# reinforcement-learning-kr/alpha_omok

Measured on AMD Instinct MI355X. Metric: self-play move-decisions/sec (9x9, 400 sims/move), higher is better.
Workload: dtype f32 (fp16x2-split MFMA operands, 3 products per multiply-add, f32 accumulate; inter-layer activations stored as two fp16 halves: ~22 significand bits)

## Files before the change

### alpha_omok_amd/csrc/net.hip

```cpp
#include <hip/hip_runtime.h>

#include <cmath>
#include <cstdio>
#include <cstdlib>
#include <cstring>
#include <map>
#include <type_traits>
#include <string>
#include <thread>
#include <vector>

#include "../../include/omok_hip.h"
#include "engine_types.hpp"
#include "host_handle.hpp"
#include "launchers.hpp"
#include "net_device.hpp"
#include "net_common.hpp"
#include "net_trunk_f32.hpp"
#include "net_trunk_h16.hpp"
#include "net_layer_ksplit.hpp"
#include "net_board_h16.hpp"
#include "net_small.hpp"
#include "net_w16.hpp"
#include "net_f16.hpp"
// ... 7 lines not shown
    int mode = 0;
    int requested_mode = 0;
    int fp16_fallbacks = 0;
    bool forced_fp32 = false;
    int num_cu = 256;
    bool finalized = false;
    std::map<std::string, std::vector<float>> params;
    ao::DevPool pool;
    std::vector<std::pair<void*, size_t>> pallocs;
    size_t pcursor = 0;
    std::vector<float*> conv_w, conv_sc, conv_sh;
    std::vector<uint4*> convh_wh, convh_wl;
    uint4 *step_w1h = nullptr, *step_w1l = nullptr;
    std::vector<float*> convh_sc;
    float* conv0_w16 = nullptr;
    float* conv0_w1 = nullptr;
    int nchq1 = 0;
    float *head_w3 = nullptr, *head_sc3 = nullptr, *head_sh3 = nullptr;
    float *wp_t = nullptr, *bp = nullptr, *w1_t = nullptr, *b1 = nullptr, *w2 = nullptr, *b2 = nullptr;
    int ws_boards = 0;
    float *act_x = nullptr, *act_t = nullptr, *hbuf = nullptr, *il_in = nullptr;
    float *tmp_p = nullptr, *tmp_v = nullptr;
    int* d_status = nullptr;
    bool attr_l[16][2] = {}, attr_done[16] = {}, lds_attr_done[16] = {}, attr_k[16] = {};
    int ksplit_min = 48, ksplit_max = 64, ksplit_max2 = 0;
    int rowk_min = 1, rowk_max = 47;
    bool attr_r[16] = {};
    int boardk_min = 64;
    bool attr_b[16] = {};
    long perboard_cells = 2592;
    int force_xt = 0, force_nch = 0;
    bool force_resident = false;
    ao::EventTimer timer{512};
    bool timing = false;
    int last_in_kind = 1;
    bool w16 = false;
    int products_req = 0;
    int precision_req = AO_NET_PRECISION_FP32;
    int trunk_fmt = -1;
};

template <typename T>
static int param_alloc(ao_net* n, T** out, size_t count) {
    const size_t bytes = std::max<size_t>(count * sizeof(T), 16);
    if (n->pcursor < n->pallocs.size() && n->pallocs[n->pcursor].second == bytes) {
        *out = static_cast<T*>(n->pallocs[n->pcursor++].first);
        return 0;
    }
    void* p = nullptr;
    hipError_t st = hipMalloc(&p, bytes);
    if (st != hipSuccess) return n->fail(std::string("hipMalloc(") + std::to_string(bytes) + " B): " + hipGetErrorString(st));
    n->pool.adopt(p);
    if (n->pcursor < n->pallocs.size()) {
        n->pool.release(n->pallocs[n->pcursor].first);
        n->pallocs[n->pcursor] = {p, bytes};
    } else {
        n->pallocs.push_back({p, bytes});
    }
    ++n->pcursor;
    *out = static_cast<T*>(p);
    return 0;
// ... 459 lines not shown
            hipLaunchKernelGGL(k_head_fc, dim3(boards), dim3(256), lds1, s, n->hbuf, n->wp_t, n->bp, n->w1_t, n->b1, n->w2, n->b2, policy, value,
                               n->A, n->planes);
            AO_HIP(n, hipGetLastError());
            return 0;
        } else {
            for (int l = 0; l <= 2 * n->nb; ++l)
                if (layer(l)) return 1;
        }
        AO_HIP(n, hipGetLastError());
        heads_h16 = f16l ? 2 : 1;
    } else if (group == 16 && mode == 5) {
        TrunkHArgs a;
        a.in0 = reinterpret_cast<const float4*>(in_il);
        a.bufA = reinterpret_cast<uint4*>(n->act_x);
        a.bufB = reinterpret_cast<uint4*>(n->act_t);
        a.nlayers = 1 + 2 * n->nb;
        a.CQ = n->CQ;
        a.COUT = n->planes;
        a.w3 = n->head_w3; a.sc3 = n->head_sc3; a.sh3 = n->head_sh3;
        a.wp_t = n->wp_t; a.bp = n->bp; a.w1_t = n->w1_t; a.b1 = n->b1; a.w2 = n->w2; a.b2 = n->b2;
        a.policy = policy;
        a.value = value;
        a.live = live; a.row_cap = row_cap;
        for (int l = 0; l < a.nlayers; ++l) {
            a.layers[l].wh = n->convh_wh[l];
            a.layers[l].wl = n->convh_wl[l];
            a.layers[l].sc = reinterpret_cast<const float4*>(n->convh_sc[l]);
            a.layers[l].sh = reinterpret_cast<const float4*>(n->conv_sh[l]);
            a.layers[l].ovf = n->d_status;
        }
        if (n->timing) n->timer.begin(s);
        if (fp16_forward(n)) {
            if (n->B > 9) return n->fail("split-fp16 trunk: board larger than 9x9");
            AO_HIP(n, ao::launch_trunk16h_f16(n->device, n->B, in_kind, groups, s, a));
        } else if (two_products(n) && n->trunk_fmt != 1) {
            if (n->B > 9) return n->fail("split-fp16 trunk: board larger than 9x9");
            AO_HIP(n, ao::launch_trunk16h_w16(n->device, n->B, in_kind, groups, s, a));
        } else
        switch (n->B) {
#define AO_BW_CASE(W)                                                                                        \
    case W: {                                                                                                \
        constexpr size_t heads_ = (static_cast<size_t>(3) * 128 + 16 * 3 * W * W + 8 * 16 * W * W + 8 * 16 * 128) * 4;  \
        constexpr size_t rows_ = static_cast<size_t>(2) * W * 4 * 2 * 1024 + 64;    \
        constexpr size_t lds_ = (rows_ > heads_) ? rows_ : heads_;                                            \
        if (!n->attr_done[W]) {                                                                                 \
            AO_HIP(n, hipFuncSetAttribute(reinterpret_cast<const void*>(&k_trunk16h<W, 4, 0>),              \
                                           hipFuncAttributeMaxDynamicSharedMemorySize, static_cast<int>(lds_))); \
            AO_HIP(n, hipFuncSetAttribute(reinterpret_cast<const void*>(&k_trunk16hb<W, 4, 0>),              \
                                           hipFuncAttributeMaxDynamicSharedMemorySize, static_cast<int>(lds_))); \
            AO_HIP(n, hipFuncSetAttribute(reinterpret_cast<const void*>(&k_trunk16h<W, 4, 1>),              \
                                           hipFuncAttributeMaxDynamicSharedMemorySize, static_cast<int>(lds_))); \
            AO_HIP(n, hipFuncSetAttribute(reinterpret_cast<const void*>(&k_trunk16hb<W, 4, 1>),              \
                                           hipFuncAttributeMaxDynamicSharedMemorySize, static_cast<int>(lds_))); \
            n->attr_done[W] = true;                                                                           \
        }                                                                                                    \
        if (n->trunk_fmt == 1) {                                                                             \
            if (in_kind == 2) hipLaunchKernelGGL((k_trunk16hb<W, 4, 1>), dim3(groups), dim3(512), lds_, s, a);    \
            else hipLaunchKernelGGL((k_trunk16h<W, 4, 1>), dim3(groups), dim3(512), lds_, s, a);                 \
        } else {                                                                                             \
            if (in_kind == 2) hipLaunchKernelGGL((k_trunk16hb<W, 4, 0>), dim3(groups), dim3(512), lds_, s, a);    \
            else hipLaunchKernelGGL((k_trunk16h<W, 4, 0>), dim3(groups), dim3(512), lds_, s, a);                 \
        }                                                                                                    \
    } break;
            AO_BW_CASE(3) AO_BW_CASE(4) AO_BW_CASE(5) AO_BW_CASE(6) AO_BW_CASE(7) AO_BW_CASE(8) AO_BW_CASE(9)
#undef AO_BW_CASE
            default: return n->fail("split-fp16 trunk: board larger than 9x9");
        }
        if (n->timing) n->timer.end(s);
        AO_HIP(n, hipGetLastError());
#ifdef AO_PROF
        if (getenv("AO_PROF_PRINT")) {
            unsigned long long h[96];
            hipStreamSynchronize(s);
            hipMemcpyFromSymbol(h, HIP_SYMBOL(ao_prof), sizeof(h));
            static const char* nm[12] = {"stage0", "slabs", "epilogue", "barrier", "last_epi+boundary", "heads", "conv1", "total",
                                         "s0:sync1", "s0:stage-issue", "s0:loads-land", "s0:sync2"};
            for (int k = 0; k < 12; ++k) {
                fprintf(stderr, "AO_PROF %-18s", nm[k]);
                for (int t = 0; t < 8; ++t) fprintf(stderr, " %9llu", h[t * 12 + k]);
// ... 118 lines not shown
    n->nchq16 = (((inplanes + 3) / 4) + 7) & ~7;
    n->nchq1 = (((inplanes + 3) / 4) + 3) & ~3;
    n->CQ = planes / 4;
    {
        hipDeviceProp_t prop;
        if (hipGetDeviceProperties(&prop, device) == hipSuccess && prop.multiProcessorCount > 0)
            n->num_cu = prop.multiProcessorCount;
    }
    if (const char* v = getenv("AO_KSPLIT")) {
        int lo = 0, hi = 0, hi2 = 0;
        if (sscanf(v, "%d,%d,%d", &lo, &hi, &hi2) == 3) { n->ksplit_min = lo > 0 ? lo : 1 << 30; n->ksplit_max = hi; n->ksplit_max2 = hi2; }
    }
    if (const char* v = getenv("AO_PERBOARD_CELLS")) n->perboard_cells = atol(v);
    if (const char* v = getenv("AO_BOARDK")) n->boardk_min = atoi(v);
    if (const char* v = getenv("AO_ROWK")) {
        int lo = 0, hi = -1;
        if (sscanf(v, "%d,%d", &lo, &hi) == 2) { n->rowk_min = lo; n->rowk_max = hi; }
    }
    if (const char* v = getenv("AO_TRUNK_FMT")) n->trunk_fmt = atoi(v) == 1 ? 1 : 0;
    if (n->trunk_fmt < 0) n->trunk_fmt = 0;
    if (const char* v = getenv("AO_XT")) n->force_xt = atoi(v) == 4 ? 4 : (atoi(v) == 5 ? 5 : 0);
    if (const char* v = getenv("AO_NCH")) n->force_nch = atoi(v) > 0 && atoi(v) <= board ? atoi(v) : 0;
    if (const char* v = getenv("AO_FORCE_RESIDENT")) n->force_resident = atoi(v) != 0;
    return 0;
}

void ao_net_destroy(ao_net* n) {
    if (!n) return;
    hipSetDevice(n->device);
    hipDeviceSynchronize();
    n->pool.free_all();
    n->timer.destroy();
    delete n;
}

int ao_net_create(int n_block, int inplanes, int planes, int board, int device, ao_net** out) {
    if (!out) return 1;
    ao_net* n = new ao_net();
    return ao::finish_create(n, net_create_impl(n, n_block, inplanes, planes, board, device), out, ao_net_destroy);
}

int ao_net_set_mode(ao_net* n, int mode) {
    if (mode < 0 || mode > 6)
        return n->fail("mode must be 0 (auto), 1 (layer kernels), 2 (group-resident trunk), 3 (per-board), 4 (row-chunked), 5 (split-fp16 trunk) "
                       "or 6 (split-fp16 per-layer kernels for every batch size)");
    if ((mode == 5 || mode == 6) && !h16_supported(n))
// ... 395 lines not shown
```

### alpha_omok_amd/csrc/net_f16.hip

```cpp
#include <hip/hip_runtime.h>

#include <cstdint>

#include "../../include/omok_hip.h"
#include "engine_types.hpp"
#include "net_device.hpp"
#include "net_common.hpp"
#include "net_trunk_f32.hpp"
#include "net_trunk_h16.hpp"
#include "net_board_h16.hpp"
#include "net_f16.hpp"

namespace ao {

#if AO_KO == 0 && AO_BKO == 0 && !AO_CONV1_SPLIT

namespace {
constexpr int kDev = 16;
bool g_attr_trunk[kDev][16][2], g_attr_board[kDev][16][2];

template <typename K>
hipError_t set_lds(bool* done, K kernel, size_t lds) {
    if (*done) return hipSuccess;
    const hipError_t st = hipFuncSetAttribute(reinterpret_cast<const void*>(kernel), hipFuncAttributeMaxDynamicSharedMemorySize, static_cast<int>(lds));
    if (st == hipSuccess) *done = true;
    return st;
}
}

hipError_t launch_trunk16h_f16(int device, int B, int in_kind, int groups, hipStream_t s, const TrunkHArgs& a) {
    if (device < 0 || device >= kDev) return hipErrorInvalidDevice;
    const int k = in_kind == 2 ? 1 : 0;
    switch (B) {
#define AO_BW_CASE(W)                                                                                                  \
    case W: {                                                                                                          \
        constexpr size_t heads_ = (static_cast<size_t>(3) * 128 + 16 * 3 * W * W + 8 * 16 * W * W + 8 * 16 * 128) * 4; \
        constexpr size_t rows_ = static_cast<size_t>(2) * W * 4 * 2 * 1024 + 64;                                       \
        constexpr size_t lds_ = (rows_ > heads_) ? rows_ : heads_;                                                     \
        hipError_t st = k ? set_lds(&g_attr_trunk[device][W][1], &k_trunk16hb_f16<W, 4, 0>, lds_)                      \
                          : set_lds(&g_attr_trunk[device][W][0], &k_trunk16h_f16<W, 4, 0>, lds_);                      \
        if (st != hipSuccess) return st;                                                                               \
        if (k) hipLaunchKernelGGL((k_trunk16hb_f16<W, 4, 0>), dim3(groups), dim3(512), lds_, s, a);                    \
        else hipLaunchKernelGGL((k_trunk16h_f16<W, 4, 0>), dim3(groups), dim3(512), lds_, s, a);                       \
    } break;
        AO_BW_CASE(3) AO_BW_CASE(4) AO_BW_CASE(5) AO_BW_CASE(6) AO_BW_CASE(7) AO_BW_CASE(8) AO_BW_CASE(9)
#undef AO_BW_CASE
        default: return hipErrorInvalidValue;
    }
    return hipGetLastError();
}

hipError_t launch_boardh_f16(int device, int B, bool bits, dim3 grid, hipStream_t s, const BoardHArgs& a) {
    if (device < 0 || device >= kDev) return hipErrorInvalidDevice;
    switch (B) {
#define AO_BW_CASE(W)                                                                                                  \
    case W: {                                                                                                          \
        constexpr size_t lds_ = static_cast<size_t>(W) * 8 * 1024;                                                     \
        hipError_t st = bits ? set_lds(&g_attr_board[device][W][1], &k_boardh_f16<W, 2>, lds_)                         \
                             : set_lds(&g_attr_board[device][W][0], &k_boardh_f16<W, 1>, lds_);                        \
        if (st != hipSuccess) return st;                                                                               \
        if (bits) hipLaunchKernelGGL((k_boardh_f16<W, 2>), grid, dim3(512), lds_, s, a);                               \
// ... 18 lines not shown
```

### alpha_omok_amd/csrc/net_trunk_h16.hpp

```cpp
#pragma once

#include <type_traits>

namespace ao {

struct TrunkHLayer {
    const uint4* wh;
    const uint4* wl;
    const float4* sc;
    const float4* sh;
    int* ovf;
};

struct TrunkHArgs {
    const float4* in0;
    uint4* bufA;
    uint4* bufB;
    int nlayers;
    int CQ, COUT;
    const float *w3, *sc3, *sh3, *wp_t, *bp, *w1_t, *b1, *w2, *b2;
    float* policy;
    float* value;
    const unsigned* live;
    unsigned row_cap;
    TrunkHLayer layers[kMaxTrunkLayers];
};

typedef unsigned int u32x2 __attribute__((ext_vector_type(2)));
__device__ __forceinline__ half8 buf_ld_h8(__amdgpu_buffer_rsrc_t r, int voff, int soff) {
    return __builtin_bit_cast(half8, __builtin_amdgcn_raw_buffer_load_b128(r, voff, soff, 0));
}
#ifndef AO_AUX_RES
#define AO_AUX_RES 0
#endif
#ifndef AO_AUX_ST
#define AO_AUX_ST 0
#endif
#ifndef AO_AUX_STAGE
#define AO_AUX_STAGE 0
#endif
__device__ __forceinline__ half4 buf_ld_h4(__amdgpu_buffer_rsrc_t r, int voff, int soff) {
    return __builtin_bit_cast(half4, __builtin_amdgcn_raw_buffer_load_b64(r, voff, soff, AO_AUX_RES));
}
__device__ __forceinline__ void buf_st_h4(half4 v, __amdgpu_buffer_rsrc_t r, int voff, int soff) {
    __builtin_amdgcn_raw_buffer_store_b64(__builtin_bit_cast(u32x2, v), r, voff, soff, AO_AUX_ST);
}

// ... 52 lines not shown
    }
    asm volatile("" ::: "memory");
}

__host__ __device__ constexpr int kPlaneRow(int bw) { return bw * bw <= 128 ? 128 : 256; }
__host__ __device__ constexpr unsigned kPairBytes(int fmt) { return fmt == 1 ? 1536u : 2048u; }

constexpr float kLo8Scale = 0x1p-112f;
__device__ __forceinline__ float lo8_scaled(unsigned h, unsigned l) { return __uint_as_float(((h << 8) | l) << 5); }
__device__ __forceinline__ unsigned lo8_word(float vs) {
    const unsigned u = __float_as_uint(vs);
    return (u + 15u + ((u >> 5) & 1u)) >> 5;
}

template <int BW, int NC32, int NCI, int KIND, int FMT = 0, int NPROD = 3>
struct TrunkHLayerFn {
static_assert(NPROD >= 1 && NPROD <= 3, "products per multiply-add: 3 (any fp32 weights), 2 (weights on the fp16 grid), 1 (fp16 forward)");
static constexpr bool W16 = NPROD <= 2;
static constexpr bool F16 = NPROD == 1;
static_assert(!F16 || (FMT == 0 && AO_KO == 0 && !AO_CONV1_SPLIT), "the one-product form exists for the 4-byte geometry only");
static __device__ __forceinline__ void run(const void* src, uint4* dst, const TrunkHLayer& L, const bool RES, uint4* s_x,
                                           int tile, int lane, unsigned long long* prof, const bool flip,
                                           unsigned* s_cnt, const unsigned rows_before, const bool hand_next, const int par,
                                           const bool to_heads = false) {
    constexpr bool FIRST = KIND != 0;
    constexpr bool BITS = KIND == 2;
    constexpr bool HAND = FMT == 0 && AO_KO == 0;
    constexpr bool HANDED = HAND && !FIRST;
    static_assert(!HAND || NC32 >= 2, "conv1's hand-off assumes that its own row buffers lie inside the next layer's buffer 0");
    constexpr bool RES1 = BITS && HAND && !AO_CONV1_SPLIT && !AO_SPLIT_BARRIER;
    static_assert(!RES1 || (BW >= 2 && BW * BW <= 2 * BW * NC32 * 2),
                  "conv1's resident board (BW*BW high-half fragments) lies inside the two row buffers of the next layer");
    auto py = [&](int y) { return flip ? BW - 1 - y : y; };
    constexpr int A = BW * BW;
    constexpr int NT = NC32 * 2;
    constexpr int NSP = 2;
    constexpr int NFR = BW * NCI * NSP;
    constexpr int NFRO = BW * NC32 * NSP;
    constexpr int NB = NCI * 3;
    constexpr int NPR = 3;
    constexpr int PAIR = static_cast<int>(kPairBytes(FMT));
    constexpr int NPAIR = BW * NCI;
    const int kq = lane >> 4, b = lane & 15;
    const int lane16 = lane * 16;
    const int out_voff = (((tile & 1) * 2 + (kq >> 1)) * 16 + b) * 16 + (kq & 1) * 8;
    float4 sc = L.sc[tile * 4 + kq], sh = L.sh[tile * 4 + kq];
    if (FMT == 1) {
        sc.x *= kLo8Scale; sc.y *= kLo8Scale; sc.z *= kLo8Scale; sc.w *= kLo8Scale;
        sh.x *= kLo8Scale; sh.y *= kLo8Scale; sh.z *= kLo8Scale; sh.w *= kLo8Scale;
    }
    const __amdgpu_buffer_rsrc_t rs_wh = make_rsrc(L.wh, 9u * NCI * NT * 1024u);
    const __amdgpu_buffer_rsrc_t rs_wl = make_rsrc(L.wl, 9u * NCI * NT * 1024u);
    const __amdgpu_buffer_rsrc_t rs_src =
// ... 28 lines not shown
                h[k] = (kq == 0 && split == 0 && ((bits >> k) & 1u)) ? static_cast<_Float16>(1.0f) : static_cast<_Float16>(0.0f);
            return h;
        }
        const int o = ((cell * 8 + 2 * kq) * 16 + b) * 16;
        const u32x4 q0 = __builtin_amdgcn_raw_buffer_load_b128(rs_src, o, 0, 0);
        const u32x4 q1 = __builtin_amdgcn_raw_buffer_load_b128(rs_src, o + 256, 0, 0);
        half8 h;
#pragma unroll
        for (int k = 0; k < 4; ++k) {
            const float v0 = __uint_as_float(q0[k]), v1 = __uint_as_float(q1[k]);
            const _Float16 h0 = static_cast<_Float16>(v0), h1 = static_cast<_Float16>(v1);
            h[k] = split ? static_cast<_Float16>(v0 - static_cast<float>(h0)) : h0;
            h[4 + k] = split ? static_cast<_Float16>(v1 - static_cast<float>(h1)) : h1;
        }
        return h;
    };
    float peak = 0.f;
    unsigned pbits[BITS ? (NFR + NT - 1) / NT : 1] = {};
    f32x4 acc[3][BW];
#pragma unroll
    for (int r = 0; r < 3; ++r)
#pragma unroll
        for (int i = 0; i < BW; ++i) acc[r][i] = f32x4{0.f, 0.f, 0.f, 0.f};
    auto epilogue = [&](int yo, auto ho, uint4* hx) {
        constexpr bool HO = decltype(ho)::value;
        constexpr int HB = (BW + 1) / 2;
#pragma unroll
        for (int i0 = 0; i0 < BW; i0 += HB) {
            half4 rh[HB], rl[HB];
            unsigned rb[HB];
            if (RES) {
#pragma unroll
                for (int k = 0; k < HB; ++k) {
                    const int i = i0 + k < BW ? i0 + k : BW - 1;
                    const int ob = ((py(yo) * BW + i) * NC32 + (tile >> 1)) * PAIR;
                    rh[k] = buf_ld_h4(rs_dst, out_voff, ob);
                    if (FMT == 1) {
                        rb[k] = __builtin_amdgcn_raw_buffer_load_b32(rs_dst, out_voff >> 1, ob + 1024, AO_AUX_RES);
                    } else if (AO_KO == 10 || AO_KO == 12) {
                        const unsigned u = __builtin_amdgcn_raw_buffer_load_b32(rs_dst, out_voff >> 1, ob + 1024, AO_AUX_RES);
                        rl[k] = __builtin_bit_cast(half4, u32x2{u, u});
                    } else if (!F16) {
                        rl[k] = buf_ld_h4(rs_dst, out_voff, ob + 1024);
                    }
                }
            }
#pragma unroll
            for (int k = 0; k < HB; ++k) {
                const int i = i0 + k;
                if (i >= BW) continue;
                const f32x4 c = acc[0][i];
                float f[4] = {fmaf(c[0], sc.x, sh.x), fmaf(c[1], sc.y, sh.y), fmaf(c[2], sc.z, sh.z), fmaf(c[3], sc.w, sh.w)};
                const int ob = ((py(yo) * BW + i) * NC32 + (tile >> 1)) * PAIR;
                if (RES) {
                    if (FMT == 1) {
                        const u32x2 hb = __builtin_bit_cast(u32x2, rh[k]);
#pragma unroll
                        for (int r = 0; r < 4; ++r)
                            f[r] += lo8_scaled((hb[r >> 1] >> (16 * (r & 1))) & 0xffffu, (rb[k] >> (8 * r)) & 0xffu);
                    } else if (F16) {
#pragma unroll
                        for (int r = 0; r < 4; ++r) f[r] += static_cast<float>(rh[k][r]);
                    } else {
#pragma unroll
                        for (int r = 0; r < 4; ++r) f[r] += static_cast<float>(rh[k][r]) + static_cast<float>(rl[k][r]);
                    }
                }
                peak = fmaxf(fmaxf(peak, fmaxf(f[0], f[1])), fmaxf(f[2], f[3]));
                if (FMT == 1) {
                    unsigned t[4];
#pragma unroll
                    for (int r = 0; r < 4; ++r)
                        t[r] = lo8_word(f[r] >= 0x1p-126f ? fminf(f[r], 65504.f * kLo8Scale) : 0.f);
                    const u32x2 hw = {(t[0] >> 8) | ((t[1] >> 8) << 16), (t[2] >> 8) | ((t[3] >> 8) << 16)};
// ... 103 lines not shown
            const int f = tile + NT * k;
            if (f < NFR && !(AO_KO == 10 && (f & 1) && lane >= 32))
                __builtin_amdgcn_raw_ptr_buffer_load_lds(rs_src, (__attribute__((address_space(3))) void*)(s_x + f * 64), 16,
                                                         (AO_KO == 12 && (f & 1) && lane >= 32) ? lane16 - 512 : lane16,
                                                         (py(0) * NFR + f) * 1024, 0, AO_AUX_STAGE);
        }
    }
    AO_T(t_a2);
    load_w(0, wA);
    if (!HANDED) asm volatile("s_waitcnt vmcnt(0) lgkmcnt(0)" ::: "memory");
    if (FMT == 1 && !FIRST) {
        expand_pairs(s_x, 0, (NPAIR + NT - 1) / NT);
        asm volatile("s_waitcnt lgkmcnt(0)" ::: "memory");
    }
    AO_T(t_a3);
    if (!HANDED) __syncthreads();
    AO_T(t_b);
    AO_ACC(0, t_a, t_b);
    AO_ACC(8, t_a, t_a1);
    AO_ACC(9, t_a1, t_a2);
    AO_ACC(10, t_a2, t_a3);
    AO_ACC(11, t_a3, t_b);

    for (int yi = 0; yi < BW; ++yi) {
        AO_T(t_r0);
        const uint4* xs = RES1 ? s_x + static_cast<size_t>(yi) * BW * 64
                               : s_x + static_cast<size_t>((yi + po) & 1) * NFR * 64;
        auto xfrag = [&](int xi, int c, int sp) {
            return __builtin_bit_cast(half8, xs[(RES1 ? xi : (xi * NCI + c) * NSP + sp) * 64 + lane]);
        };
        uint4* xn = s_x + static_cast<size_t>((yi + 1 + po) & 1) * NFR * 64;
        const int yn = yi + 1;
        const bool stage_next = !RES1 && yn < BW && !(HANDED && yi == 0);
#pragma unroll
        for (int slab = 0; slab < NB; ++slab) {
            const int c = slab / 3, dy = slab % 3;
            half8 (&w)[2][3] = (slab & 1) ? wB : wA;
            half8 (&wn)[2][3] = (slab & 1) ? wA : wB;
            {
                const int ty = slab + 1 < NB ? yi : yi + 1, tyo = ty + 1 - (slab + 1) % 3;
                load_w(slab + 1, wn, ty < BW && tyo >= 0 && tyo < BW);
            }
            if (!stage_next) {
            } else if (dy == 1 && !AO_KO_NOSTAGE && FMT == 1 && !FIRST) {
                constexpr int K2 = (NPAIR / NT + NCI - 1) / (NCI > 1 ? NCI - 1 : 1);
                if (c > 0 && AO_KO != 11) expand_pairs(xn, (c - 1) * K2, c * K2);
// ... 91 lines not shown
        for (int i = 0; i < BW; ++i) {
            acc[0][i] = acc[1][i];
            acc[1][i] = acc[2][i];
            acc[2][i] = f32x4{0.f, 0.f, 0.f, 0.f};
        }
        AO_T(t_r2);
#if AO_SPLIT_BARRIER
        if ((yi + 1 < BW || (HAND && hand_next)) && AO_KO != 9) row_wait(s_cnt, static_cast<unsigned>(NT) * (rows_before + static_cast<unsigned>(yi) + 1u));
#else
        if (RES1) {}
        else if (AO_KO == 9) asm volatile("s_waitcnt vmcnt(0) lgkmcnt(0)" ::: "memory");
        else asm volatile("s_waitcnt vmcnt(0) lgkmcnt(0)\n\ts_barrier" ::: "memory");
#endif
        AO_T(t_r3);
        AO_ACC(1, t_r0, t_r1);
        AO_ACC(2, t_r1, t_r2);
        AO_ACC(3, t_r2, t_r3);
    }
    AO_T(t_c);
    if (!AO_KO_NOEPI || FIRST) {
        if (HAND && hand_next) epilogue(BW - 1, kHand, hand1);
        else epilogue(BW - 1, kStore, nullptr);
    }
    if (peak > (FMT == 1 ? 65504.f * kLo8Scale : 65504.f)) atomicOr(L.ovf, 1);
    asm volatile("s_waitcnt vmcnt(0)" ::: "memory");
    __syncthreads();
    __builtin_amdgcn_fence(__ATOMIC_ACQUIRE, "workgroup");
    AO_T(t_d);
    AO_ACC(4, t_c, t_d);
}
};

template <int BW, int XT, int NC32, int NCI, int KIND, int NPROD = 3>
__device__ __forceinline__ void trunk_h_layer_tile(const void* src, uint4* dst, const TrunkHLayer& L, const bool RES,
                                                   uint4* s_x, int tile, int lane, int x0, int yb, int ye) {
    static_assert(NPROD >= 1 && NPROD <= 3, "products per multiply-add: 3 (any fp32 weights), 2 (weights on the fp16 grid), 1 (fp16 forward)");
    constexpr bool W16 = NPROD <= 2;
    constexpr bool F16 = NPROD == 1;
    static_assert(!F16 || (AO_KO == 0 && !AO_CONV1_SPLIT), "the one-product form is no timing experiment");
    constexpr bool FIRST = KIND != 0;
    constexpr bool BITS = KIND == 2;
    constexpr int A = BW * BW;
    constexpr bool HALO = XT < BW;
    constexpr int NX = HALO ? XT + 2 : XT;
    constexpr int NT = NC32 * 2;
    constexpr int NSP = 2;
    constexpr int NFR = NX * NCI * NSP;
    constexpr int NB = NCI * 3;
    constexpr int NPR = 3;
    const int kq = lane >> 4, b = lane & 15;
    const int lane16 = lane * 16;
    const int out_voff = (((tile & 1) * 2 + (kq >> 1)) * 16 + b) * 16 + (kq & 1) * 8;
// ... 220 lines not shown
                                               a.layer, false, s_x, tile, lane, xt * XT, yb, ye);
    } else if (KIND == 1) {
        trunk_h_layer_tile<BW, XT, NC32, 1, 1, NPROD>(static_cast<const float4*>(a.src) + static_cast<size_t>(grp) * A * 8 * 16, dst, a.layer,
                                               false, s_x, tile, lane, xt * XT, yb, ye);
    } else {
        trunk_h_layer_tile<BW, XT, NC32, NC32, 0, NPROD>(static_cast<const uint4*>(a.src) + static_cast<size_t>(grp) * A * NC32 * 2 * 64, dst,
                                                      a.layer, a.res != 0, s_x, tile, lane, xt * XT, yb, ye);
    }
}

template <int BW, int XT, int NC32, int KIND>
__global__ __launch_bounds__(NC32 * 2 * 64, 1) void k_layer16h(LayerHArgs a) {
    layer16h_body<BW, XT, NC32, KIND, 3>(a);
}
template <int BW, int XT, int NC32, int KIND>
__global__ __launch_bounds__(NC32 * 2 * 64, 1) void k_layer16h_w16(LayerHArgs a) {
    layer16h_body<BW, XT, NC32, KIND, 2>(a);
}
template <int BW, int XT, int NC32, int KIND>
__global__ __launch_bounds__(NC32 * 2 * 64, 1) void k_layer16h_f16(LayerHArgs a) {
    layer16h_body<BW, XT, NC32, KIND, 1>(a);
}

template <int BW, int NC32, int INK, int FMT, int NPROD = 3>
__device__ __forceinline__ void trunk16h_body(const TrunkHArgs& a) {
    static_assert(FMT == 0 || AO_SPLIT_BARRIER == 0, "the split row barrier is implemented for the 4-byte format only");
    constexpr int A = BW * BW;
    extern __shared__ __attribute__((aligned(16))) uint4 s_x[];
    const int grp = blockIdx.x;
    if (grp >= live_groups16(a.live, a.row_cap, grp + 1)) return;
    const int lane = threadIdx.x & 63;
    const int tile = __builtin_amdgcn_readfirstlane(static_cast<int>(threadIdx.x) >> 6);
    const size_t gq = static_cast<size_t>(AO_KO == 5 ? grp % 64 : AO_KO == 6 ? grp % 128 : grp) * A * NC32 * (kPairBytes(FMT) / 16);
    uint4* bufA = a.bufA + gq;
    uint4* bufB = a.bufB + gq;
    unsigned long long prof[12] = {0, 0, 0, 0, 0, 0, 0, 0, 0, 0, 0, 0};
    unsigned long long* pp = prof;
    unsigned* s_cnt = reinterpret_cast<unsigned*>(s_x + static_cast<size_t>(2) * BW * NC32 * 2 * 64);
    if (threadIdx.x == 0) *s_cnt = 0u;
    const bool ko_fill = AO_KO == 13 || AO_KO == 15;
    AO_T(t0);
    if (INK == 2)
        TrunkHLayerFn<BW, NC32, 1, 2, FMT, NPROD>::run(reinterpret_cast<const uint8_t*>(a.in0) + static_cast<size_t>(grp) * 16 * kPlaneRow(BW), bufA,
                                      a.layers[0], false, s_x, tile, lane, pp, false, s_cnt, 0u, a.nlayers > 1, 0);
    else
        TrunkHLayerFn<BW, NC32, 1, 1, FMT, NPROD>::run(a.in0 + static_cast<size_t>(grp) * A * 8 * 16, bufA, a.layers[0], false, s_x, tile, lane, pp, false,
                                      s_cnt, 0u, a.nlayers > 1, 0);
    AO_T(t1);
    if (ko_fill) {
        __syncthreads();
        for (int f = tile; f < 2 * BW * NC32 * 2; f += NC32 * 2) s_x[f * 64 + lane] = ao_ko_fragment((grp * 4u * BW * NC32 + f) * 64u + lane, f & 1);
        __syncthreads();
    }
#ifdef AO_PROF
    for (int k = 0; k < 12; ++k) prof[k] = 0;
#endif
    static_assert(2 * BW * 16 <= NC32 * 2 * 64, "trunk_heads gives every (cell, board) of the two handed rows a thread of its own");
    const bool to_heads = FMT == 0 && AO_KO == 0 && a.nlayers > 1;
    int par = 0;
    for (int l = 1; l < a.nlayers; ++l) {
        const bool second = (l & 1) == 0;
        TrunkHLayerFn<BW, NC32, NC32, 0, FMT, NPROD>::run(second ? bufB : bufA, second ? bufA : bufB, a.layers[l], second, s_x, tile, lane, pp,
                                             (l & 1) != 0, s_cnt, static_cast<unsigned>(l) * BW, l + 1 < a.nlayers || to_heads, par,
                                             to_heads && l + 1 == a.nlayers);
        par = (par + BW - 1) & 1;
    }
    AO_T(t2);
    constexpr size_t kRowQ = static_cast<size_t>(BW) * NC32 * 2 * 64;
    if (AO_KO != 8)
        trunk_heads<BW, FMT == 1 ? 2 : NPROD == 1 ? 3 : 1>(a, reinterpret_cast<const float4*>(a.bufA), static_cast<size_t>(grp) * A, grp,
                                          to_heads ? s_x + (par ^ 1) * kRowQ : nullptr, to_heads ? s_x + par * kRowQ : nullptr);
#ifdef AO_PROF
    AO_T(t3);
    prof[5] = t3 - t2;
    prof[6] = t1 - t0;
    prof[7] = t3 - t0;
    if (grp == 5 && lane == 0)
        for (int k = 0; k < 12; ++k) ao_prof[tile * 12 + k] = prof[k];
#endif
}

template <int BW, int NC32, int FMT>
__global__ __launch_bounds__(NC32 * 2 * 64, 1) void k_trunk16h(TrunkHArgs a) {
    trunk16h_body<BW, NC32, 1, FMT>(a);
}
template <int BW, int NC32, int FMT>
__global__ __launch_bounds__(NC32 * 2 * 64, 1) void k_trunk16hb(TrunkHArgs a) {
    trunk16h_body<BW, NC32, 2, FMT>(a);
}
template <int BW, int NC32, int FMT>
__global__ __launch_bounds__(NC32 * 2 * 64, 1) void k_trunk16h_w16(TrunkHArgs a) {
    trunk16h_body<BW, NC32, 1, FMT, 2>(a);
}
template <int BW, int NC32, int FMT>
__global__ __launch_bounds__(NC32 * 2 * 64, 1) void k_trunk16hb_w16(TrunkHArgs a) {
    trunk16h_body<BW, NC32, 2, FMT, 2>(a);
}
template <int BW, int NC32, int FMT>
__global__ __launch_bounds__(NC32 * 2 * 64, 1) void k_trunk16h_f16(TrunkHArgs a) {
    trunk16h_body<BW, NC32, 1, FMT, 1>(a);
}
template <int BW, int NC32, int FMT>
__global__ __launch_bounds__(NC32 * 2 * 64, 1) void k_trunk16hb_f16(TrunkHArgs a) {
    trunk16h_body<BW, NC32, 2, FMT, 1>(a);
}

}
```

### alpha_omok_amd/csrc/net_w16.hip

```cpp
#include <hip/hip_runtime.h>

#include <cstdint>

#include "../../include/omok_hip.h"
#include "engine_types.hpp"
#include "net_device.hpp"
#include "net_common.hpp"
#include "net_trunk_f32.hpp"
#include "net_trunk_h16.hpp"
#include "net_layer_ksplit.hpp"
#include "net_board_h16.hpp"
#include "net_w16.hpp"

namespace ao {

namespace {
constexpr int kDev = 16;
bool g_attr_trunk[kDev][16][2], g_attr_layer[kDev][16][2], g_attr_board[kDev][16][2], g_attr_ksplit[kDev][16][2];

template <typename K>
hipError_t set_lds(bool* done, K kernel, size_t lds) {
    if (*done) return hipSuccess;
    const hipError_t st = hipFuncSetAttribute(reinterpret_cast<const void*>(kernel), hipFuncAttributeMaxDynamicSharedMemorySize, static_cast<int>(lds));
    if (st == hipSuccess) *done = true;
    return st;
}
}

hipError_t launch_trunk16h_w16(int device, int B, int in_kind, int groups, hipStream_t s, const TrunkHArgs& a) {
    if (device < 0 || device >= kDev) return hipErrorInvalidDevice;
    const int k = in_kind == 2 ? 1 : 0;
    switch (B) {
#define AO_BW_CASE(W)                                                                                                  \
    case W: {                                                                                                          \
        constexpr size_t heads_ = (static_cast<size_t>(3) * 128 + 16 * 3 * W * W + 8 * 16 * W * W + 8 * 16 * 128) * 4; \
        constexpr size_t rows_ = static_cast<size_t>(2) * W * 4 * 2 * 1024 + 64;                                       \
        constexpr size_t lds_ = (rows_ > heads_) ? rows_ : heads_;                                                     \
        hipError_t st = k ? set_lds(&g_attr_trunk[device][W][1], &k_trunk16hb_w16<W, 4, 0>, lds_)                      \
                          : set_lds(&g_attr_trunk[device][W][0], &k_trunk16h_w16<W, 4, 0>, lds_);                      \
        if (st != hipSuccess) return st;                                                                               \
        if (k) hipLaunchKernelGGL((k_trunk16hb_w16<W, 4, 0>), dim3(groups), dim3(512), lds_, s, a);                    \
        else hipLaunchKernelGGL((k_trunk16h_w16<W, 4, 0>), dim3(groups), dim3(512), lds_, s, a);                       \
    } break;
        AO_BW_CASE(3) AO_BW_CASE(4) AO_BW_CASE(5) AO_BW_CASE(6) AO_BW_CASE(7) AO_BW_CASE(8) AO_BW_CASE(9)
#undef AO_BW_CASE
        default: return hipErrorInvalidValue;
    }
    return hipGetLastError();
}

hipError_t launch_layer16h_w16(int device, int B, int xt, dim3 grid, hipStream_t s, const LayerHArgs& a) {
    if (device < 0 || device >= kDev) return hipErrorInvalidDevice;
#define AO_LAYERH_LAUNCH(W, XT_)                                                                                       \
    do {                                                                                                               \
        constexpr int NX_ = (XT_ < W) ? XT_ + 2 : XT_;                                                                 \
        constexpr size_t lds_ = static_cast<size_t>(2) * NX_ * 4 * 2 * 1024;                                           \
        const hipError_t st = set_lds(&g_attr_layer[device][W][XT_ == 4], &k_layer16h_w16<W, XT_, 4, 0>, lds_);        \
        if (st != hipSuccess) return st;                                                                               \
        hipLaunchKernelGGL((k_layer16h_w16<W, XT_, 4, 0>), grid, dim3(512), lds_, s, a);                               \
    } while (0)
// ... 71 lines not shown
```

Measured before the change: 6909.

## Pair output rows in trunk conv to share each weight slab across two rows

Adds a row-pair schedule to the split-fp16 trunk conv layer. Each weight slab loaded from memory now feeds MFMAs for two input rows at once, with staging and barriers planned by a compile-time phase table in a new header. The goal is to cut the number of weight slab loads and barriers per layer. Because the kernels pass `pairs = !ROWS` and ROWS defaults to false, the paired path is the default; setting AO_TRUNK_ROWLOOP switches back to the old per-row loop. The cost is more complex barrier and staging logic and higher register pressure from keeping several row accumulators live.

```diff
diff --git a/alpha_omok_amd/csrc/net.hip b/alpha_omok_amd/csrc/net.hip
--- a/alpha_omok_amd/csrc/net.hip
+++ b/alpha_omok_amd/csrc/net.hip
@@ -53,7 +53,7 @@
     float *act_x = nullptr, *act_t = nullptr, *hbuf = nullptr, *il_in = nullptr;
     float *tmp_p = nullptr, *tmp_v = nullptr;
     int* d_status = nullptr;
-    bool attr_l[16][2] = {}, attr_done[16] = {}, lds_attr_done[16] = {}, attr_k[16] = {};
+    bool attr_l[16][2] = {}, attr_done[16] = {}, attr_rows[16] = {}, lds_attr_done[16] = {}, attr_k[16] = {};
     int ksplit_min = 48, ksplit_max = 64, ksplit_max2 = 0;
     int rowk_min = 1, rowk_max = 47;
     bool attr_r[16] = {};
@@ -68,6 +68,7 @@
     bool w16 = false;
     int products_req = 0;
     int precision_req = AO_NET_PRECISION_FP32;
+    bool trunk_rowloop = false;
     int trunk_fmt = -1;
 };
 
@@ -573,6 +574,7 @@
         a.policy = policy;
         a.value = value;
         a.live = live; a.row_cap = row_cap;
+        a.rowloop = n->trunk_rowloop ? 1 : 0;
         for (int l = 0; l < a.nlayers; ++l) {
             a.layers[l].wh = n->convh_wh[l];
             a.layers[l].wl = n->convh_wl[l];
@@ -605,7 +607,18 @@
                                            hipFuncAttributeMaxDynamicSharedMemorySize, static_cast<int>(lds_))); \
             n->attr_done[W] = true;                                                                           \
         }                                                                                                    \
-        if (n->trunk_fmt == 1) {                                                                             \
+        constexpr bool R_ = W >= ao::kRowPairMinBW;    \
+        if (R_ && a.rowloop && n->trunk_fmt != 1) {                                                          \
+            if (!n->attr_rows[W]) {                                                                           \
+                AO_HIP(n, hipFuncSetAttribute(reinterpret_cast<const void*>(&k_trunk16h<W, 4, 0, R_>),      \
+                                               hipFuncAttributeMaxDynamicSharedMemorySize, static_cast<int>(lds_))); \
+                AO_HIP(n, hipFuncSetAttribute(reinterpret_cast<const void*>(&k_trunk16hb<W, 4, 0, R_>),     \
+                                               hipFuncAttributeMaxDynamicSharedMemorySize, static_cast<int>(lds_))); \
+                n->attr_rows[W] = true;                                                                       \
+            }                                                                                                \
+            if (in_kind == 2) hipLaunchKernelGGL((k_trunk16hb<W, 4, 0, R_>), dim3(groups), dim3(512), lds_, s, a); \
+            else hipLaunchKernelGGL((k_trunk16h<W, 4, 0, R_>), dim3(groups), dim3(512), lds_, s, a);             \
+        } else if (n->trunk_fmt == 1) {                                                                      \
             if (in_kind == 2) hipLaunchKernelGGL((k_trunk16hb<W, 4, 1>), dim3(groups), dim3(512), lds_, s, a);    \
             else hipLaunchKernelGGL((k_trunk16h<W, 4, 1>), dim3(groups), dim3(512), lds_, s, a);                 \
         } else {                                                                                             \
@@ -770,6 +783,7 @@
     if (const char* v = getenv("AO_XT")) n->force_xt = atoi(v) == 4 ? 4 : (atoi(v) == 5 ? 5 : 0);
     if (const char* v = getenv("AO_NCH")) n->force_nch = atoi(v) > 0 && atoi(v) <= board ? atoi(v) : 0;
     if (const char* v = getenv("AO_FORCE_RESIDENT")) n->force_resident = atoi(v) != 0;
+    if (const char* v = getenv("AO_TRUNK_ROWLOOP")) n->trunk_rowloop = atoi(v) != 0;
     return 0;
 }
 
diff --git a/alpha_omok_amd/csrc/net_f16.hip b/alpha_omok_amd/csrc/net_f16.hip
--- a/alpha_omok_amd/csrc/net_f16.hip
+++ b/alpha_omok_amd/csrc/net_f16.hip
@@ -17,7 +17,7 @@
 
 namespace {
 constexpr int kDev = 16;
-bool g_attr_trunk[kDev][16][2], g_attr_board[kDev][16][2];
+bool g_attr_trunk[kDev][16][2], g_attr_trunk_rows[kDev][16][2], g_attr_board[kDev][16][2];
 
 template <typename K>
 hipError_t set_lds(bool* done, K kernel, size_t lds) {
@@ -37,6 +37,15 @@
         constexpr size_t heads_ = (static_cast<size_t>(3) * 128 + 16 * 3 * W * W + 8 * 16 * W * W + 8 * 16 * 128) * 4; \
         constexpr size_t rows_ = static_cast<size_t>(2) * W * 4 * 2 * 1024 + 64;                                       \
         constexpr size_t lds_ = (rows_ > heads_) ? rows_ : heads_;                                                     \
+        constexpr bool R_ = W >= kRowPairMinBW;    \
+        if (R_ && a.rowloop) {                                                                                         \
+            hipError_t st = k ? set_lds(&g_attr_trunk_rows[device][W][1], &k_trunk16hb_f16<W, 4, 0, R_>, lds_)         \
+                              : set_lds(&g_attr_trunk_rows[device][W][0], &k_trunk16h_f16<W, 4, 0, R_>, lds_);         \
+            if (st != hipSuccess) return st;                                                                           \
+            if (k) hipLaunchKernelGGL((k_trunk16hb_f16<W, 4, 0, R_>), dim3(groups), dim3(512), lds_, s, a);            \
+            else hipLaunchKernelGGL((k_trunk16h_f16<W, 4, 0, R_>), dim3(groups), dim3(512), lds_, s, a);               \
+            break;                                                                                                     \
+        }                                                                                                              \
         hipError_t st = k ? set_lds(&g_attr_trunk[device][W][1], &k_trunk16hb_f16<W, 4, 0>, lds_)                      \
                           : set_lds(&g_attr_trunk[device][W][0], &k_trunk16h_f16<W, 4, 0>, lds_);                      \
         if (st != hipSuccess) return st;                                                                               \
diff --git a/alpha_omok_amd/csrc/net_trunk_h16.hpp b/alpha_omok_amd/csrc/net_trunk_h16.hpp
--- a/alpha_omok_amd/csrc/net_trunk_h16.hpp
+++ b/alpha_omok_amd/csrc/net_trunk_h16.hpp
@@ -1,6 +1,8 @@
 #pragma once
 
 #include <type_traits>
+
+#include "trunk_row_schedule.hpp"
 
 namespace ao {
 
@@ -23,6 +25,7 @@
     float* value;
     const unsigned* live;
     unsigned row_cap;
+    int rowloop;
     TrunkHLayer layers[kMaxTrunkLayers];
 };
 
@@ -121,13 +124,14 @@
 static __device__ __forceinline__ void run(const void* src, uint4* dst, const TrunkHLayer& L, const bool RES, uint4* s_x,
                                            int tile, int lane, unsigned long long* prof, const bool flip,
                                            unsigned* s_cnt, const unsigned rows_before, const bool hand_next, const int par,
-                                           const bool to_heads = false) {
+                                           const bool to_heads = false, const bool pairs = false) {
     constexpr bool FIRST = KIND != 0;
     constexpr bool BITS = KIND == 2;
     constexpr bool HAND = FMT == 0 && AO_KO == 0;
     constexpr bool HANDED = HAND && !FIRST;
     static_assert(!HAND || NC32 >= 2, "conv1's hand-off assumes that its own row buffers lie inside the next layer's buffer 0");
     constexpr bool RES1 = BITS && HAND && !AO_CONV1_SPLIT && !AO_SPLIT_BARRIER;
+    constexpr bool PAIRABLE = KIND == 0 && HAND && !AO_SPLIT_BARRIER && BW >= kRowPairMinBW;
     static_assert(!RES1 || (BW >= 2 && BW * BW <= 2 * BW * NC32 * 2),
                   "conv1's resident board (BW*BW high-half fragments) lies inside the two row buffers of the next layer");
     auto py = [&](int y) { return flip ? BW - 1 - y : y; };
@@ -202,7 +206,7 @@
     for (int r = 0; r < 3; ++r)
 #pragma unroll
         for (int i = 0; i < BW; ++i) acc[r][i] = f32x4{0.f, 0.f, 0.f, 0.f};
-    auto epilogue = [&](int yo, auto ho, uint4* hx) {
+    auto epilogue = [&](int yo, auto ho, uint4* hx, int sl = 0) {
         constexpr bool HO = decltype(ho)::value;
         constexpr int HB = (BW + 1) / 2;
 #pragma unroll
@@ -229,7 +233,7 @@
             for (int k = 0; k < HB; ++k) {
                 const int i = i0 + k;
                 if (i >= BW) continue;
-                const f32x4 c = acc[0][i];
+                const f32x4 c = acc[sl][i];
                 float f[4] = {fmaf(c[0], sc.x, sh.x), fmaf(c[1], sc.y, sh.y), fmaf(c[2], sc.z, sh.z), fmaf(c[3], sc.w, sh.w)};
                 const int ob = ((py(yo) * BW + i) * NC32 + (tile >> 1)) * PAIR;
                 if (RES) {
@@ -379,6 +383,153 @@
     AO_ACC(10, t_a2, t_a3);
     AO_ACC(11, t_a3, t_b);
 
+    bool paired = false;
+    if constexpr (PAIRABLE) {
+    if (pairs) {
+        static_assert(NCI % 2 == 0 && NCI == NC32, "phases of an even number of slabs: the weight double buffer's parity carries over");
+        constexpr int FP = row_full_periods(BW);
+        constexpr int NPH = row_phases(BW);
+        constexpr int TAIL_DY = row_phase(BW, row_next_phase(BW, 3 * FP - 1)).dy;
+        static_assert(FP >= 1 && row_next_phase(BW, 3 * FP - 1) >= 0 && row_phase(BW, 1).stage_row == 2 && row_phase(BW, 2).stage_row == 3,
+                      "the first period is a full one that stages in both of its staging phases, and a shorter period follows the full ones");
+        constexpr int NSPS = F16 ? 1 : 2;
+        constexpr int H = NCI / 2;
+        static_assert(row_stage_blocks(H - 1, NCI).c0 == 0 && row_stage_blocks(H - 1, NCI).c1 == H && row_stage_blocks(NCI - 1, NCI).c0 == H &&
+                      row_stage_blocks(NCI - 1, NCI).c1 == NCI, "the two staging points of a phase");
+        uint4* const xe = s_x + static_cast<size_t>(po) * NFR * 64;
+        uint4* const xo = s_x + static_cast<size_t>(po ^ 1) * NFR * 64;
+        int q64 = 64 * 64;
+        asm volatile("" : "+v"(q64));
+        const int lane_hi = q64 + lane;
+        auto stage_blocks = [&](int row, uint4* xb, auto c0_, auto c1_) __attribute__((always_inline)) {
+            constexpr int c0 = decltype(c0_)::value, c1 = decltype(c1_)::value;
+            constexpr int nf = BW * (c1 - c0) * NSPS;
+#pragma unroll
+            for (int k = 0; k < (nf + NT - 1) / NT; ++k) {
+                const int j = tile + NT * k;
+                if (j < nf) {
+                    const int f = ((j / (NSPS * (c1 - c0))) * NCI + c0 + (j / NSPS) % (c1 - c0)) * NSP + j % NSPS;
+                    __builtin_amdgcn_raw_ptr_buffer_load_lds(rs_src, (__attribute__((address_space(3))) void*)(xb + f * 64), 16, lane16,
+                                                             (py(row) * NFR + f) * 1024, 0, AO_AUX_STAGE);
+                }
+            }
+        };
+        auto half_slab = [&](const uint4* xs, int sl, int c, half8 (&w)[2][3]) __attribute__((always_inline)) {
+            auto xfrag = [&](int xi, int sp) {
+                const int f = (xi * NCI + c) * NSP + sp;
+                return __builtin_bit_cast(half8, xs[f < 64 ? f * 64 + lane : (f - 64) * 64 + lane_hi]);
+            };
+            half8 xh = xfrag(0, 0);
+            half8 xl = F16 ? xh : xfrag(0, 1);
+#pragma unroll
+            for (int xi = 0; xi < BW; ++xi) {
+                half8 nh = xh, nl = xl;
+                if (xi + 1 < BW) {
+                    nh = xfrag(xi + 1, 0);
+                    nl = F16 ? nh : xfrag(xi + 1, 1);
+                }
+#pragma unroll
+                for (int pr = 0; pr < NPR; ++pr) {
+                    if (W16 && pr == 1) continue;
+                    if (F16 && pr == 2) continue;
+#pragma unroll
+                    for (int dx = 0; dx < 3; ++dx) {
+                        const int i = xi - dx + 1;
+                        if (i < 0 || i >= BW) continue;
+                        acc[sl][i] = __builtin_amdgcn_mfma_f32_16x16x32_f16(w[pr == 1 ? 1 : 0][dx], pr == 2 ? xl : xh, acc[sl][i], 0, 0, 0);
+                    }
+                }
+                xh = nh;
+                xl = nl;
+                __builtin_amdgcn_sched_barrier(0);
+            }
+        };
+        auto phase = [&](const int k, const int dy, const bool on0, const bool on1, const int sl0, const int sl1, const int b0, const int b1,
+                         const int nslab, const bool nissued) __attribute__((always_inline)) {
+            const int srow = row_phase(BW, k).stage_row;
+#pragma unroll
+            for (int c = 0; c < NCI; ++c) {
+                half8 (&w)[2][3] = (c & 1) ? wB : wA;
+                half8 (&wn)[2][3] = (c & 1) ? wA : wB;
+                if (c + 1 < NCI) load_w((c + 1) * 3 + dy, wn);
+                else load_w(nslab, wn, nissued);
+                if (on0) half_slab(b0 ? xo : xe, sl0, c, w);
+                if (on1) half_slab(b1 ? xo : xe, sl1, c, w);
+                __builtin_amdgcn_sched_barrier(0);
+                if ((c == H - 1 || c == NCI - 1) && !row_barrier_behind_epilogues(dy, c, NCI) && row_barrier_after(BW, k, c, NCI)) {
+                    AO_T(t_b0);
+                    asm volatile("s_waitcnt vmcnt(0) lgkmcnt(0)\n\ts_barrier" ::: "memory");
+                    AO_T(t_b1);
+                    AO_ACC(3, t_b0, t_b1);
+                    AO_ACC(1, t_b1, t_b0);
+                    if (srow >= 0 && c == H - 1) stage_blocks(srow, b0 ? xo : xe, std::integral_constant<int, 0>{}, std::integral_constant<int, H>{});
+                    if (srow >= 0 && c == NCI - 1) stage_blocks(srow, b0 ? xo : xe, std::integral_constant<int, H>{}, std::integral_constant<int, NCI>{});
+                }
+            }
+        };
+        for (int p = 0; p < FP; ++p) {
+            const int k = 3 * p, a = 2 * p;
+            AO_T(t_r0);
+            phase(k, 0, true, true, 1, 2, 0, 1, 1, true);
+            phase(k + 1, 1, true, true, 0, 1, 0, 1, 2, true);
+            phase(k + 2, 2, true, true, 0, 1, 1, 0, p + 1 < FP ? 0 : TAIL_DY, true);
+            AO_T(t_r1);
+            epilogue(a, kStore, nullptr, 0);
+            __builtin_amdgcn_sched_barrier(0);
+            if (a + 1 < BW - 2) {
+                epilogue(a + 1, kStore, nullptr, 1);
+#pragma unroll
+                for (int i = 0; i < BW; ++i) acc[1][i] = f32x4{0.f, 0.f, 0.f, 0.f};
+            }
+#pragma unroll
+            for (int i = 0; i < BW; ++i) {
+                acc[0][i] = acc[2][i];
+                acc[2][i] = f32x4{0.f, 0.f, 0.f, 0.f};
+            }
+            AO_T(t_r2);
+            static_assert(row_barrier_behind_epilogues(2, NCI - 1, NCI), "the barrier the third phase left out");
+            if (row_barrier_after(BW, k + 2, NCI - 1, NCI)) {
+                asm volatile("s_waitcnt vmcnt(0) lgkmcnt(0)\n\ts_barrier" ::: "memory");
+                stage_blocks(a + 3, xo, std::integral_constant<int, H>{}, std::integral_constant<int, NCI>{});
+            }
+            AO_T(t_r3);
+            AO_ACC(1, t_r0, t_r1);
+            AO_ACC(2, t_r1, t_r2);
+            AO_ACC(3, t_r2, t_r3);
+        }
+        {
+            AO_T(t_r0);
+#pragma unroll
+            for (int k = 3 * FP; k < NPH; ++k) {
+                const RowPhase ph = row_phase(BW, k);
+                if (!ph.h[0].on && !ph.h[1].on) continue;
+                const int kn = row_next_phase(BW, k);
+                phase(k, ph.dy, ph.h[0].on, ph.h[1].on, ph.h[0].slot, ph.h[1].slot, ph.h[0].buf, ph.h[1].buf, kn >= 0 ? row_phase(BW, kn).dy : 0,
+                      kn >= 0);
+            }
+            AO_T(t_r1);
+            AO_ACC(1, t_r0, t_r1);
+        }
+        {
+            AO_T(t_e0);
+            constexpr int S2 = row_final_slot(BW - 2);
+            if (HAND && hand_next) {
+                asm volatile("s_waitcnt lgkmcnt(0)\n\ts_barrier" ::: "memory");
+                epilogue(BW - 2, kHand, hand2, S2);
+                __builtin_amdgcn_sched_barrier(0);
+                epilogue(BW - 1, kHand, hand1, S2 ^ 1);
+            } else {
+                epilogue(BW - 2, kStore, nullptr, S2);
+                __builtin_amdgcn_sched_barrier(0);
+                epilogue(BW - 1, kStore, nullptr, S2 ^ 1);
+            }
+            AO_T(t_e1);
+            AO_ACC(4, t_e0, t_e1);
+        }
+        paired = true;
+    }
+    }
+    if (!paired) {
     for (int yi = 0; yi < BW; ++yi) {
         AO_T(t_r0);
         const uint4* xs = RES1 ? s_x + static_cast<size_t>(yi) * BW * 64
@@ -516,12 +667,16 @@
         if (HAND && hand_next) epilogue(BW - 1, kHand, hand1);
         else epilogue(BW - 1, kStore, nullptr);
     }
+    AO_T(t_c1);
+    AO_ACC(4, t_c, t_c1);
+    }
+    AO_T(t_c2);
     if (peak > (FMT == 1 ? 65504.f * kLo8Scale : 65504.f)) atomicOr(L.ovf, 1);
     asm volatile("s_waitcnt vmcnt(0)" ::: "memory");
     __syncthreads();
     __builtin_amdgcn_fence(__ATOMIC_ACQUIRE, "workgroup");
     AO_T(t_d);
-    AO_ACC(4, t_c, t_d);
+    AO_ACC(4, t_c2, t_d);
 }
 };
 
@@ -788,7 +943,7 @@
     layer16h_body<BW, XT, NC32, KIND, 1>(a);
 }
 
-template <int BW, int NC32, int INK, int FMT, int NPROD = 3>
+template <int BW, int NC32, int INK, int FMT, int NPROD = 3, bool ROWS = false>
 __device__ __forceinline__ void trunk16h_body(const TrunkHArgs& a) {
     static_assert(FMT == 0 || AO_SPLIT_BARRIER == 0, "the split row barrier is implemented for the 4-byte format only");
     constexpr int A = BW * BW;
@@ -828,7 +983,7 @@
         const bool second = (l & 1) == 0;
         TrunkHLayerFn<BW, NC32, NC32, 0, FMT, NPROD>::run(second ? bufB : bufA, second ? bufA : bufB, a.layers[l], second, s_x, tile, lane, pp,
                                              (l & 1) != 0, s_cnt, static_cast<unsigned>(l) * BW, l + 1 < a.nlayers || to_heads, par,
-                                             to_heads && l + 1 == a.nlayers);
+                                             to_heads && l + 1 == a.nlayers, !ROWS);
         par = (par + BW - 1) & 1;
     }
     AO_T(t2);
@@ -846,29 +1001,29 @@
 #endif
 }
 
-template <int BW, int NC32, int FMT>
+template <int BW, int NC32, int FMT, bool ROWS = false>
 __global__ __launch_bounds__(NC32 * 2 * 64, 1) void k_trunk16h(TrunkHArgs a) {
-    trunk16h_body<BW, NC32, 1, FMT>(a);
-}
-template <int BW, int NC32, int FMT>
+    trunk16h_body<BW, NC32, 1, FMT, 3, ROWS>(a);
+}
+template <int BW, int NC32, int FMT, bool ROWS = false>
 __global__ __launch_bounds__(NC32 * 2 * 64, 1) void k_trunk16hb(TrunkHArgs a) {
-    trunk16h_body<BW, NC32, 2, FMT>(a);
-}
-template <int BW, int NC32, int FMT>
+    trunk16h_body<BW, NC32, 2, FMT, 3, ROWS>(a);
+}
+template <int BW, int NC32, int FMT, bool ROWS = false>
 __global__ __launch_bounds__(NC32 * 2 * 64, 1) void k_trunk16h_w16(TrunkHArgs a) {
-    trunk16h_body<BW, NC32, 1, FMT, 2>(a);
-}
-template <int BW, int NC32, int FMT>
+    trunk16h_body<BW, NC32, 1, FMT, 2, ROWS>(a);
+}
+template <int BW, int NC32, int FMT, bool ROWS = false>
 __global__ __launch_bounds__(NC32 * 2 * 64, 1) void k_trunk16hb_w16(TrunkHArgs a) {
-    trunk16h_body<BW, NC32, 2, FMT, 2>(a);
-}
-template <int BW, int NC32, int FMT>
+    trunk16h_body<BW, NC32, 2, FMT, 2, ROWS>(a);
+}
+template <int BW, int NC32, int FMT, bool ROWS = false>
 __global__ __launch_bounds__(NC32 * 2 * 64, 1) void k_trunk16h_f16(TrunkHArgs a) {
-    trunk16h_body<BW, NC32, 1, FMT, 1>(a);
-}
-template <int BW, int NC32, int FMT>
+    trunk16h_body<BW, NC32, 1, FMT, 1, ROWS>(a);
+}
+template <int BW, int NC32, int FMT, bool ROWS = false>
 __global__ __launch_bounds__(NC32 * 2 * 64, 1) void k_trunk16hb_f16(TrunkHArgs a) {
-    trunk16h_body<BW, NC32, 2, FMT, 1>(a);
-}
-
-}
+    trunk16h_body<BW, NC32, 2, FMT, 1, ROWS>(a);
+}
+
+}
diff --git a/alpha_omok_amd/csrc/net_w16.hip b/alpha_omok_amd/csrc/net_w16.hip
--- a/alpha_omok_amd/csrc/net_w16.hip
+++ b/alpha_omok_amd/csrc/net_w16.hip
@@ -16,7 +16,7 @@
 
 namespace {
 constexpr int kDev = 16;
-bool g_attr_trunk[kDev][16][2], g_attr_layer[kDev][16][2], g_attr_board[kDev][16][2], g_attr_ksplit[kDev][16][2];
+bool g_attr_trunk[kDev][16][2], g_attr_trunk_rows[kDev][16][2], g_attr_layer[kDev][16][2], g_attr_board[kDev][16][2], g_attr_ksplit[kDev][16][2];
 
 template <typename K>
 hipError_t set_lds(bool* done, K kernel, size_t lds) {
@@ -36,6 +36,15 @@
         constexpr size_t heads_ = (static_cast<size_t>(3) * 128 + 16 * 3 * W * W + 8 * 16 * W * W + 8 * 16 * 128) * 4; \
         constexpr size_t rows_ = static_cast<size_t>(2) * W * 4 * 2 * 1024 + 64;                                       \
         constexpr size_t lds_ = (rows_ > heads_) ? rows_ : heads_;                                                     \
+        constexpr bool R_ = W >= kRowPairMinBW;    \
+        if (R_ && a.rowloop) {                                                                                         \
+            hipError_t st = k ? set_lds(&g_attr_trunk_rows[device][W][1], &k_trunk16hb_w16<W, 4, 0, R_>, lds_)         \
+                              : set_lds(&g_attr_trunk_rows[device][W][0], &k_trunk16h_w16<W, 4, 0, R_>, lds_);         \
+            if (st != hipSuccess) return st;                                                                           \
+            if (k) hipLaunchKernelGGL((k_trunk16hb_w16<W, 4, 0, R_>), dim3(groups), dim3(512), lds_, s, a);            \
+            else hipLaunchKernelGGL((k_trunk16h_w16<W, 4, 0, R_>), dim3(groups), dim3(512), lds_, s, a);               \
+            break;                                                                                                     \
+        }                                                                                                              \
         hipError_t st = k ? set_lds(&g_attr_trunk[device][W][1], &k_trunk16hb_w16<W, 4, 0>, lds_)                      \
                           : set_lds(&g_attr_trunk[device][W][0], &k_trunk16h_w16<W, 4, 0>, lds_);                      \
         if (st != hipSuccess) return st;                                                                               \
diff --git a/alpha_omok_amd/csrc/trunk_row_schedule.hpp b/alpha_omok_amd/csrc/trunk_row_schedule.hpp
--- /dev/null
+++ b/alpha_omok_amd/csrc/trunk_row_schedule.hpp
@@ -0,0 +1,94 @@
+#pragma once
+
+#if defined(__HIPCC__)
+#define AO_SCHED_HD __host__ __device__
+#else
+#define AO_SCHED_HD
+#endif
+
+namespace ao {
+
+constexpr int kRowPairMinBW = 4;
+
+struct RowHalf {
+    bool on;
+    int row;
+    int out;
+    int slot;
+    int buf;
+};
+struct RowPhase {
+    int dy;
+    RowHalf h[2];
+    int stage_row;
+    int done[2];
+};
+
+AO_SCHED_HD constexpr int row_periods(int bw) { return (bw + 1) / 2; }
+AO_SCHED_HD constexpr int row_phases(int bw) { return 3 * row_periods(bw); }
+
+AO_SCHED_HD constexpr RowPhase row_phase(int bw, int k) {
+    const int a = 2 * (k / 3), dy = k % 3;
+    const int r0 = dy == 2 ? a + 1 : a, r1 = r0 + 1;
+    const int o0 = r0 + 1 - dy, o1 = r1 + 1 - dy;
+    RowPhase p{dy,
+               {{r0 < bw && o0 < bw, r0, o0, o0 - a, r0 & 1}, {r1 < bw && o1 < bw, r1, o1, o1 - a, r1 & 1}},
+               -1,
+               {-1, -1}};
+    if (dy == 1 && a + 2 < bw) p.stage_row = a + 2;
+    if (dy == 2 && a + 3 < bw) p.stage_row = a + 3;
+    if (dy == 2) {
+        p.done[0] = a;
+        p.done[1] = a + 1 < bw ? a + 1 : -1;
+    }
+    return p;
+}
+AO_SCHED_HD constexpr bool row_phase_on(int bw, int k) { return row_phase(bw, k).h[0].on || row_phase(bw, k).h[1].on; }
+
+AO_SCHED_HD constexpr bool row_period_full(int bw, int p) {
+    for (int k = 3 * p; k < 3 * p + 3; ++k)
+        if (!row_phase(bw, k).h[0].on || !row_phase(bw, k).h[1].on) return false;
+    return true;
+}
+AO_SCHED_HD constexpr int row_full_periods(int bw) {
+    int n = 0;
+    while (n < row_periods(bw) && row_period_full(bw, n)) ++n;
+    return n;
+}
+
+AO_SCHED_HD constexpr int row_next_phase(int bw, int k) {
+    for (int n = k + 1; n < row_phases(bw); ++n)
+        if (row_phase_on(bw, n)) return n;
+    return -1;
+}
+
+struct BlockRange { int c0, c1; };
+AO_SCHED_HD constexpr BlockRange row_stage_blocks(int c, int nci) {
+    const int h = nci / 2;
+    if (c == h - 1) return {0, h};
+    if (c == nci - 1) return {h, nci};
+    return {0, 0};
+}
+AO_SCHED_HD constexpr BlockRange row_stage_after(int bw, int k, int c, int nci) {
+    if (row_phase(bw, k).stage_row < 0) return {0, 0};
+    return row_stage_blocks(c, nci);
+}
+AO_SCHED_HD constexpr bool row_barrier_after(int bw, int k, int c, int nci) {
+    const BlockRange s = row_stage_after(bw, k, c, nci);
+    if (s.c0 != s.c1) return true;
+    return c == nci / 2 - 1 && k > 0 && row_phase(bw, k - 1).stage_row >= 0;
+}
+
+AO_SCHED_HD constexpr bool row_barrier_behind_epilogues(int dy, int c, int nci) { return dy == 2 && c == nci - 1; }
+
+AO_SCHED_HD constexpr int row_epilogue_after(int bw, int yo) { return yo >= bw - 2 ? row_phases(bw) - 1 : 3 * (yo / 2) + 2; }
+AO_SCHED_HD constexpr int row_final_slot(int yo) { return yo & 1; }
+
+AO_SCHED_HD constexpr int row_pair_slab_loads(int bw, int nci) {
+    int n = 0;
+    for (int k = 0; k < row_phases(bw); ++k) n += row_phase_on(bw, k) ? nci : 0;
+    return n;
+}
+AO_SCHED_HD constexpr int row_loop_slab_loads(int bw, int nci) { return (3 * bw - 2) * nci; }
+
+}
```

Result: no change. 6966 (median of 6 runs) (+0.8%).
